# ethan-li-coding/AD-Census

Hardware: NVIDIA H100
Metric: disparity-maps/sec (450x375x64) (higher is better)
Workload: dtype f32

## Files before the change

### adcensus_b200/csrc/adc_common.cuh

```cuda
#pragma once
#include <cuda.h>
#include <cuda_runtime.h>
#include <stdint.h>

#include "img_format.h"

#define ADC_INVALID_F (__int_as_float(0x7f800000))
#define ADC_LARGE_F 99999.0f
#define ADC_CNT 16

struct AdcDims {
    int W, H, D, Dp;
    int dmin, dmax;
    int N;
    long long vol_stride;
};

struct AdcParams {
    AdcDims dm;
    int L1, L2, t1, t2;
    float p1, p2, p1_4, p2_4, p1_10, p2_10;
    int tso;
    int irv_ts; float irv_th;
    float lr_thres;
// ... 34 lines not shown
}
inline void adc_once_done(AdcOnce& o) {
    int dev = 0;
    cudaGetDevice(&dev);
    o.done[dev & 63].store(1, std::memory_order_release);
}

inline int adc_sm_count() {
    int dev = 0, n = 0;
    cudaGetDevice(&dev);
    cudaDeviceGetAttribute(&n, cudaDevAttrMultiProcessorCount, dev);
    return n > 0 ? n : 1;
}

struct alignas(64) AdcArmTmaps { unsigned char map[2][2][128]; };
struct alignas(64) AdcSoTmaps { unsigned char cost[2][2][128]; unsigned char rec[2][128]; int T[2], NS[2]; unsigned smem[2]; };
typedef CUresult (*AdcTmapEncodeFn)(CUtensorMap*, CUtensorMapDataType, cuuint32_t, void*, const cuuint64_t*, const cuuint64_t*,
                                    const cuuint32_t*, const cuuint32_t*, CUtensorMapInterleave, CUtensorMapSwizzle,
                                    CUtensorMapL2promotion, CUtensorMapFloatOOBfill);
AdcTmapEncodeFn adc_tmap_encoder();

struct AdcWave {
    int S;
    uint8_t* bgr;
    unsigned* bgrx;
    uint8_t* gray;
    unsigned long long* census;
    float* volA; float* volB;
    uchar4* arms;
    const AdcArmTmaps* arm_tm;
    unsigned* arm_rec;
    uint16_t* sup_h; uint16_t* sup_v;
    uint8_t* dmap;
    float* disp_l; float* disp_r; float* disp_t;
    uint8_t* label; uint8_t* flag;
    int* pend;
    int* vlist;
    int* counters;
    int* rowcnt;
    unsigned* so_bitrows;
    unsigned* so_rec;
    const AdcSoTmaps* so_tm;
    int* vote_work;
    int2* vote_chg;
    uchar2* vote_alr;
    uchar2* vote_atbT;
    int* vote_pslotT;
    uint16_t* vote_val;
    uint8_t* vote_dirtyb;
    int* vote_state;
    int* vote_off;
    unsigned* vote_hist;
    const float* lut_ad;
    const float* lut_cen;
    const double* ray_sin; const double* ray_cos;
    const short2* ray_off;
};
// ... 42 lines not shown
                        const uint16_t* sup, cudaStream_t st, unsigned long long* launches);
void adc_launch_arm_sum2(const AdcParams& P, const AdcWave& w, const float* src, float* dst, int dir,
                         const uint16_t* sup_mid, cudaStream_t st, unsigned long long* launches);
bool adc_cost_arm_sum_h_available(const AdcParams& P);
bool adc_launch_cost_arm_sum_h(const AdcParams& P, const AdcWave& w, float* dst, float* cost_out, cudaStream_t st,
                               unsigned long long* launches);
size_t adc_arm_rec_bytes(const AdcDims& dm, int L1);
bool adc_arm_tmaps_encode(const AdcParams& P, int S, float* volA, float* volB, AdcArmTmaps* out);
size_t adc_arm_overread_floats(const AdcDims& dm);
void adc_launch_so_bitrows(const AdcParams& P, const AdcWave& w, cudaStream_t st, unsigned long long* launches);
size_t adc_so_rec_bytes(const AdcDims& dm);
size_t adc_so_bitrow_bytes(const AdcDims& dm);
bool adc_so_tmaps_encode(const AdcParams& P, int S, float* volA, float* volB, unsigned* so_rec, AdcSoTmaps* out);
int adc_launch_scanline(const AdcParams& P, const AdcWave& w, const float* src, float* dst, int sx, int sy,
                        cudaStream_t st, unsigned long long* launches);
int adc_launch_wta(const AdcParams& P, const AdcWave& w, const float* vol, cudaStream_t st, unsigned long long* launches);
int adc_launch_scanline_wta(const AdcParams& P, const AdcWave& w, const float* src, float* rec, cudaStream_t st,
                            unsigned long long* launches);
int adc_launch_wta_merge(const AdcParams& P, const AdcWave& w, const float* rec, cudaStream_t st, unsigned long long* launches);
void adc_launch_confidence(const AdcParams& P, const AdcWave& w, const float* vol, float* min_cost, float* peak_ratio,
                           cudaStream_t st, unsigned long long* launches);
void adc_launch_outlier(const AdcParams& P, const AdcWave& w, cudaStream_t st, unsigned long long* launches);
void adc_launch_build_lists(const AdcParams& P, const AdcWave& w, cudaStream_t st, unsigned long long* launches);
void adc_launch_active_lists(const AdcParams& P, const AdcWave& w, cudaStream_t st, unsigned long long* launches);
void adc_launch_voting(const AdcParams& P, const AdcWave& w, cudaStream_t st, unsigned long long* launches);
void adc_launch_interp_list(const AdcParams& P, const AdcWave& w, int k, cudaStream_t st, unsigned long long* launches);
void adc_launch_discontinuity(const AdcParams& P, const AdcWave& w, const float* vol, cudaStream_t st, unsigned long long* launches);
int adc_launch_render(const AdcDims& dm, const float* d_disp, unsigned* d_mm, uint8_t* d_gray, uint8_t* d_jet, float* d_mm_out,
                      cudaStream_t st, unsigned long long* launches);
void adc_launch_cloud(const AdcParams& P, const AdcWave& w1, const float* d_disp, const uint8_t* d_bgr, float* d_cloud,
// ... 4 lines not shown
```

### adcensus_b200/csrc/engine.cu

```cuda
#include <cuda_runtime.h>

#include <float.h>
#include <math.h>
#include <stdarg.h>
#include <stddef.h>
#include <stdio.h>
#include <stdlib.h>
#include <string.h>

#include <algorithm>
#include <string>
#include <vector>

#include "../../include/adcensus_b200.h"
#include "adc_common.cuh"
#include "ca_plan.h"
#include "so_plan.h"

static_assert(sizeof(adc_option) == 60, "adc_option must match the reference's ADCensusOption (60 bytes)");
static_assert(offsetof(adc_option, so_p1) == 32 && offsetof(adc_option, irv_th) == 48 &&
              offsetof(adc_option, do_lr_check) == 56 && offsetof(adc_option, do_discontinuity_adjustment) == 58,
              "adc_option field offsets must match adcensus_types.h:45-75");
static_assert(sizeof(adc_image_desc) == 32 && offsetof(adc_image_desc, reserved) == 4 &&
              offsetof(adc_image_desc, row_pitch) == 8 && offsetof(adc_image_desc, plane_pitch) == 16 &&
// ... 123 lines not shown
    t.pend = c.take<int>((size_t)S * 2 * N);
    t.vlist = c.take<int>((size_t)S * 2 * N);
    t.counters = c.take<int>((size_t)S * ADC_CNT);
    t.vote_alr = c.take<uchar2>((size_t)S * N);
    t.vote_chg = c.take<int2>((size_t)S * N);
    t.vote_atbT = c.take<uchar2>((size_t)S * N);
    t.vote_pslotT = c.take<int>((size_t)S * N);
    t.vote_val = c.take<uint16_t>((size_t)S * N);
    t.vote_dirtyb = c.take<uint8_t>((size_t)S * N);
    t.vote_state = c.take<int>((size_t)S * N);
    t.vote_off = c.take<int>((size_t)S * (N + 1));
    t.rowcnt = c.take<int>((size_t)S * 2 * dm.H);
    t.so_bitrows = c.take<unsigned>((size_t)S * adc_so_bitrow_bytes(dm) / 4);
    t.so_rec = c.take<unsigned>((size_t)S * adc_so_rec_bytes(dm) / 4);
    t.vote_work = c.take<int>((size_t)S * N);
    t.vote_hist = reinterpret_cast<unsigned*>(t.volB);
    if (w) *w = t;
    return c.off;
}

void build_params(adc_engine* e) {
    const adc_option& o = e->opt;
    AdcParams& P = e->P;
    P.dm.W = e->W; P.dm.H = e->H;
    P.dm.dmin = o.min_disparity; P.dm.dmax = o.max_disparity;
    P.dm.D = o.max_disparity - o.min_disparity;
    P.dm.Dp = (P.dm.D + 3) / 4 * 4;
    P.dm.N = e->W * e->H;
    P.dm.vol_stride = (long long)P.dm.N * P.dm.Dp;
    P.L1 = std::min(o.cross_L1, 255);
// ... 209 lines not shown
    }
    if ((rc = launched("aggregation"))) return rc;
    if (ev) CK(cudaEventRecord(ev[2], st));
    if (last_stage <= ADC_STAGE_AGG4) return ADC_OK;

    adc_launch_diffmaps(P, w, st, L);
    adc_launch_so_bitrows(P, w, st, L);
    SoVolumeUse vol_use{};
    for (int i = 0; i < outs.n; i++) vol_use.opt_export |= outs.o[i].stage == ADC_VOL_OPT;
    vol_use.confidence = maps.dst[ADC_MAP_MIN_COST] || maps.dst[ADC_MAP_PEAK_RATIO];
    vol_use.discontinuity = e->opt.do_discontinuity_adjustment != 0;
    vol_use.debug_run = debug_run || last_stage < ADC_STAGE_WTA;
    const int wta_force = (e->cfg.debug_flags & ADC_DBG_UNFUSED_SO_WTA) ? SO_WTA_NEVER
                          : (e->cfg.debug_flags & ADC_DBG_FUSED_SO_WTA) ? SO_WTA_ALWAYS : SO_WTA_AUTO;
    const bool so_wta = so_wta_fused(vol_use, wta_force, P.dm.W, P.dm.H, P.dm.D, P.dm.Dp, P.dm.dmin, P.dm.vol_stride);
    static const int dirs[4][2] = {{1, 0}, {-1, 0}, {0, 1}, {0, -1}};
    for (int ps = 0; ps < 4; ps++) {
        const float* src = (ps % 2 == 0) ? A : B;
        float* dst = (ps % 2 == 0) ? B : A;
        if (ps == 3 && so_wta ? adc_launch_scanline_wta(P, w, src, dst, st, L)
                              : adc_launch_scanline(P, w, src, dst, dirs[ps][0], dirs[ps][1], st, L))
            return fail(ADC_ERR_UNSUPPORTED, "scanline pass not launched (disparity range %d, limit 256)", P.dm.D);
        if (ps % 2 == 0) e->dbg_init = B; else e->dbg_aggr = ps == 3 && so_wta ? nullptr : A;
        if (ps == 3) e->dbg_so_wta = so_wta;
        if (ps == 3) export_vol(ADC_VOL_OPT, A);
        if (stop(ADC_STAGE_SO1 + ps)) return launched("scanline optimisation");
    }
    if ((rc = launched("scanline optimisation"))) return rc;
    if (ev) CK(cudaEventRecord(ev[3], st));

    if (so_wta) adc_launch_wta_merge(P, w, A, st, L);
    else if (adc_launch_wta(P, w, A, st, L)) return fail(ADC_ERR_UNSUPPORTED, "WTA launch failed");
    if (maps.dst[ADC_MAP_WTA_LEFT])
        CK(cudaMemcpyAsync(maps.dst[ADC_MAP_WTA_LEFT], w.disp_l, mapN * sizeof(float), cudaMemcpyDeviceToDevice, st));
    if (maps.dst[ADC_MAP_WTA_RIGHT])
        CK(cudaMemcpyAsync(maps.dst[ADC_MAP_WTA_RIGHT], w.disp_r, mapN * sizeof(float), cudaMemcpyDeviceToDevice, st));
    if (maps.dst[ADC_MAP_MIN_COST] || maps.dst[ADC_MAP_PEAK_RATIO])
        adc_launch_confidence(P, w, A, static_cast<float*>(maps.dst[ADC_MAP_MIN_COST]),
// ... 1331 lines not shown
            case 16:
            case 17: {
                const long long plane = so_wta_plane(P.dm.W, P.dm.H, P.dm.D, P.dm.Dp);
                if (SO_WTA_FIELDS * plane > P.dm.vol_stride)
                    return fail(ADC_ERR_UNSUPPORTED, "adc_profile_kernel: the WTA records do not fit in a pair's volume");
                const double recs = 4.0 * SO_WTA_FIELDS * P.dm.H * (double)so_wta_row_records(P.dm.W, P.dm.D, P.dm.Dp, P.dm.dmin);
                if (kernel_id == 16) {
                    if (adc_launch_scanline_wta(P, w, w.volA, w.volB, ln.st, &e->launches)) return fail(ADC_ERR_UNSUPPORTED, "scanline");
                    bytes = V + 6 * N + recs + 4 * N;
                } else {
                    adc_launch_wta_merge(P, w, w.volB, ln.st, &e->launches);
                    bytes = recs + 4 * N;
                }
                break;
            }
            default: return fail(ADC_ERR_ARG, "adc_profile_kernel: unknown kernel id %d", kernel_id);
        }
    }
    CK(cudaEventRecord(e1, ln.st));
    CK(cudaStreamSynchronize(ln.st));
    float ms = 0;
    CK(cudaEventElapsedTime(&ms, e0, e1));
    *avg_ms = ms / reps;
    if (algorithmic_bytes) *algorithmic_bytes = bytes * e->S;
    return ADC_OK;
}

int adc_debug_run(adc_engine* e, const uint8_t* img_left, const uint8_t* img_right, int32_t last_stage) {
    const char* fn = "adc_debug_run";
    if (!e) return fail(ADC_ERR_ARG, "%s: engine is NULL", fn);
// ... 93 lines not shown
```

### adcensus_b200/csrc/k_scanline.cu

```cuda
#include "adc_common.cuh"
#include "so_plan.h"
#include <cuda.h>
#include <string.h>

template <int K>
struct Piece { static constexpr int G = (K % 4 == 0) ? 4 : ((K % 2 == 0) ? 2 : 1); static constexpr int NP = K / G; };

template <int K>
__device__ __forceinline__ void ld_vec(const float* p, int lane, int Dp, float (&v)[K]) {
    constexpr int G = Piece<K>::G, NP = Piece<K>::NP;
#pragma unroll
    for (int j = 0; j < NP; j++) {
        const int d = lane * K + j * G;
        if (d < Dp) {
            if (G == 4) { const float4 t = *reinterpret_cast<const float4*>(p + d); v[j*G] = t.x; v[j*G+1] = t.y; v[j*G+2] = t.z; v[j*G+3] = t.w; }
            else if (G == 2) { const float2 t = *reinterpret_cast<const float2*>(p + d); v[j*G] = t.x; v[j*G+1] = t.y; }
            else v[j] = p[d];
        } else {
#pragma unroll
            for (int g = 0; g < G; g++) v[j * G + g] = 0.f;
        }
    }
}

// ... 100 lines not shown
}
__device__ __forceinline__ void mbar_wait(unsigned bar, unsigned parity) {
    unsigned ok, spins = 0;
    do {
        asm volatile("{\n\t.reg .pred p;\n\tmbarrier.try_wait.parity.shared::cta.b64 p, [%1], %2;\n\tselp.u32 %0, 1, 0, p;\n\t}"
                     : "=r"(ok) : "r"(bar), "r"(parity) : "memory");
        if (!ok && ++spins > (1u << 24)) __trap();
    } while (!ok);
}
__device__ __forceinline__ void tma_load_4d(unsigned dst, const CUtensorMap* map, int c0, int c1, int c2, int c3, unsigned bar) {
    asm volatile("cp.async.bulk.tensor.4d.shared::cluster.global.tile.mbarrier::complete_tx::bytes [%0], [%1, {%2, %3, %4, %5}], [%6];"
                 ::"r"(dst), "l"(reinterpret_cast<unsigned long long>(map)), "r"(c0), "r"(c1), "r"(c2), "r"(c3), "r"(bar)
                 : "memory");
}

template <int K, int LPS, bool FULL, bool WTA>
__device__ __forceinline__ void so_pass(const CUtensorMap& tm_cost, const CUtensorMap& tm_rec, const AdcParams& P,
                                        float* __restrict__ dst, float* __restrict__ disp_l, int sx, int sy, int T, int NS) {
    constexpr int LPW = 32 / LPS;
    if constexpr (WTA) { sx = 0; sy = -1; }
    extern __shared__ __align__(128) unsigned char so_smem[];
    const AdcDims& dm = P.dm;
    const int lane = threadIdx.x & 31, wid = threadIdx.x >> 5;
    const int sub = lane / LPS, gl = lane % LPS;
    const int line0 = (blockIdx.x * SO_WARPS + wid) * LPW;
    const int line = line0 + sub;
    const int pair = blockIdx.y;
    const int n_lines = sx ? dm.H : dm.W, n_steps = sx ? dm.W : dm.H;
    if (line0 >= n_lines) return;
    const bool live = line < n_lines;
// ... 150 lines not shown
    }
#pragma unroll
    for (int o = LPS / 2; o >= 1; o >>= 1) minL = fminf(minL, __shfl_xor_sync(0xffffffffu, minL, o));
    if constexpr (WTA) {
        wta_left(row, L, minL, 0);
        wta_advance(0);
    }

    for (int step = 1; step < n_steps; step++) {
        float C[K];
        bool a1;
        unsigned bits;
        row = fetch(C, a1, bits);
        pi += pstep;

        const float up = __shfl_up_sync(0xffffffffu, L[K - 1], 1, LPS);
        const float down = __shfl_down_sync(0xffffffffu, L[0], 1, LPS);
        const float left_in = gl == 0 ? ADC_LARGE_F : up;
        const float right_in = gl == LPS - 1 ? ADC_LARGE_F : down;
        const float P1a = a1 ? P.p1 : P.p1_4, P1b = a1 ? P.p1_4 : P.p1_10;
        const float P2a = a1 ? P.p2 : P.p2_4, P2b = a1 ? P.p2_4 : P.p2_10;
        const float m4a = __fadd_rn(minL, P2a), m4b = __fadd_rn(minL, P2b);

        float Ln[K];
        float mn = ADC_LARGE_F;
#pragma unroll
        for (int k = 0; k < K; k++) {
            const bool a2 = (bits >> k) & 1u;
            const float P1 = a2 ? P1a : P1b;
            const float l1 = L[k];
            const float l2 = __fadd_rn(k > 0 ? L[k - 1] : left_in, P1);
            const float l3 = __fadd_rn(k < K - 1 ? L[k + 1] : right_in, P1);
            const float l4 = a2 ? m4a : m4b;
            float v = __fadd_rn(C[k], fminf(fminf(l1, l2), fminf(l3, l4)));
            v = __fmul_rn(v, 0.5f);
            Ln[k] = v;
            if (valid[k]) mn = fminf(mn, v);
        }
        if constexpr (WTA) {
            if constexpr (FULL && K == 8) {
                const int b = (gl >> 2) & 1;
                const float4 lo = make_float4(Ln[0], Ln[1], Ln[2], Ln[3]), hi = make_float4(Ln[4], Ln[5], Ln[6], Ln[7]);
                *reinterpret_cast<float4*>(row + 8 * gl + 4 * b) = b ? hi : lo;
                *reinterpret_cast<float4*>(row + 8 * gl + 4 - 4 * b) = b ? lo : hi;
            } else st_vec<K>(row, gl, Dp, Ln);
        } else if (live) st_vec<K>(O + (size_t)pi * Dp, gl, Dp, Ln);
#pragma unroll
        for (int k = 0; k < K; k++) L[k] = valid[k] ? Ln[k] : ADC_LARGE_F;
#pragma unroll
        for (int o = LPS / 2; o >= 1; o >>= 1) mn = fminf(mn, __shfl_xor_sync(0xffffffffu, mn, o));
        minL = mn;
        if constexpr (WTA) {
            wta_left(row, Ln, mn, step);
// ... 2 lines not shown
    }
}

template <int K, int LPS, bool FULL>
__global__ void __launch_bounds__(SO_WARPS * 32, SO_MIN_CTAS)
k_scanline(const __grid_constant__ CUtensorMap tm_cost, const __grid_constant__ CUtensorMap tm_rec, AdcParams P,
           float* __restrict__ dst, int sx, int sy, int T, int NS) {
    so_pass<K, LPS, FULL, false>(tm_cost, tm_rec, P, dst, nullptr, sx, sy, T, NS);
}

template <int K, int LPS, bool FULL>
__global__ void __launch_bounds__(SO_WARPS * 32, SO_MIN_CTAS)
k_scanline_wta(const __grid_constant__ CUtensorMap tm_cost, const __grid_constant__ CUtensorMap tm_rec, AdcParams P,
               float* __restrict__ rec, float* __restrict__ disp_l, int T, int NS) {
    so_pass<K, LPS, FULL, true>(tm_cost, tm_rec, P, rec, disp_l, 0, -1, T, NS);
}

template <int K, int LPS, bool FULL>
constexpr bool so_wta_built() { return LPS != 32 && !(K == 1 && FULL); }

template <int K, int LPS, bool FULL, bool WTA>
static int launch_scanline_kf(const AdcParams& P, const AdcWave& w, const CUtensorMap& tc, const CUtensorMap& tr,
                              int T, int NS, size_t smem, float* dst, int sx, int sy, cudaStream_t st) {
    if constexpr (WTA && !so_wta_built<K, LPS, FULL>()) {
        return 1;
    } else {
        constexpr int LPW = 32 / LPS;
        const int n_lines = sx ? P.dm.H : P.dm.W;
        const void* fn;
        if constexpr (WTA) fn = (const void*)k_scanline_wta<K, LPS, FULL>;
// ... 45 lines not shown
                    CU_TENSOR_MAP_SWIZZLE_NONE, CU_TENSOR_MAP_L2_PROMOTION_L2_256B, CU_TENSOR_MAP_FLOAT_OOB_FILL_NONE) != CUDA_SUCCESS)
                return false;
            memcpy(out->cost[v][axis], &tm, 128);
        }
        {
            const cuuint64_t gdim[4] = {(cuuint64_t)nrec, (cuuint64_t)dm.W, (cuuint64_t)dm.H, (cuuint64_t)S * 4};
            const cuuint64_t gstr[3] = {(cuuint64_t)nrec * 4, (cuuint64_t)dm.W * nrec * 4, (cuuint64_t)dm.N * nrec * 4};
            const cuuint32_t box[4] = {(cuuint32_t)nrec, bx, by, 1};
            CUtensorMap tm;
            if (enc(&tm, CU_TENSOR_MAP_DATA_TYPE_UINT32, 4, so_rec, gdim, gstr, box, estr, CU_TENSOR_MAP_INTERLEAVE_NONE,
                    CU_TENSOR_MAP_SWIZZLE_NONE, CU_TENSOR_MAP_L2_PROMOTION_L2_256B, CU_TENSOR_MAP_FLOAT_OOB_FILL_NONE) != CUDA_SUCCESS)
                return false;
            memcpy(out->rec[axis], &tm, 128);
        }
    }
    return true;
}

template <bool WTA>
static int launch_scanline(const AdcParams& P, const AdcWave& w, const float* src, float* dst, int sx, int sy,
                           cudaStream_t st, unsigned long long* launches) {
    const int Dp = P.dm.Dp;
    if (Dp > 256 || !w.so_tm || (src != w.volA && src != w.volB)) return 1;
    const int axis = sx ? 0 : 1;
    CUtensorMap tc, tr;
    memcpy(&tc, w.so_tm->cost[src == w.volB ? 1 : 0][axis], 128);
    memcpy(&tr, w.so_tm->rec[axis], 128);
    const int T = w.so_tm->T[axis], NS = w.so_tm->NS[axis];
    const size_t smem = w.so_tm->smem[axis];
    int rc = 1;
#define SO_GO(KK, LL) rc = (P.dm.D == KK * LL ? launch_scanline_kf<KK, LL, true, WTA>(P, w, tc, tr, T, NS, smem, dst, sx, sy, st) \
                                                  : launch_scanline_kf<KK, LL, false, WTA>(P, w, tc, tr, T, NS, smem, dst, sx, sy, st))
    switch (so_lanes_per_line(Dp)) {
        case 8:
            switch ((Dp + 7) / 8) { case 1: SO_GO(1, 8); break; case 2: SO_GO(2, 8); break; case 3: SO_GO(3, 8); break; case 4: SO_GO(4, 8); break;
                                    case 5: SO_GO(5, 8); break; case 6: SO_GO(6, 8); break; case 7: SO_GO(7, 8); break; default: SO_GO(8, 8); }
            break;
        case 16:
            switch ((Dp + 15) / 16) { case 5: SO_GO(5, 16); break; case 6: SO_GO(6, 16); break; case 7: SO_GO(7, 16); break; default: SO_GO(8, 16); }
            break;
        default:
            switch ((Dp + 31) / 32) { case 5: SO_GO(5, 32); break; case 6: SO_GO(6, 32); break; case 7: SO_GO(7, 32); break; default: SO_GO(8, 32); }
    }
#undef SO_GO
    if (rc) return rc;
    ++*launches;
    return 0;
}

int adc_launch_scanline(const AdcParams& P, const AdcWave& w, const float* src, float* dst, int sx, int sy,
                        cudaStream_t st, unsigned long long* launches) {
    return launch_scanline<false>(P, w, src, dst, sx, sy, st, launches);
}

int adc_launch_scanline_wta(const AdcParams& P, const AdcWave& w, const float* src, float* rec, cudaStream_t st,
                            unsigned long long* launches) {
    return launch_scanline<true>(P, w, src, rec, 0, -1, st, launches);
}

size_t adc_so_rec_bytes(const AdcDims& dm) { return (size_t)4 * dm.N * so_rec_words(dm.Dp) * 4; }
size_t adc_so_bitrow_bytes(const AdcDims& dm) { return (size_t)4 * dm.H * so_row_words(dm.W) * 4; }
```

### adcensus_b200/csrc/so_plan.h

```cpp
#pragma once
#include <stddef.h>

#ifdef __CUDACC__
#define SO_HD __host__ __device__
#else
#define SO_HD
#endif

#define SO_WARPS 4
#define SO_MIN_CTAS 8
#define SO_SMEM_MAX (160 * 1024)

SO_HD inline int so_rec_words(int Dp) { return ((1 + (Dp + 31) / 32 + 1) + 3) / 4 * 4; }
SO_HD inline int so_lanes_per_line(int Dp) { return Dp <= 64 ? 8 : (Dp <= 128 ? 16 : 32); }
SO_HD inline unsigned so_region(unsigned bytes) { return (bytes + 127u) / 128u * 128u; }
SO_HD inline unsigned so_cost_region(int Dp, int T) { return so_region((unsigned)(T * (32 / so_lanes_per_line(Dp)) * Dp * 4)); }
SO_HD inline unsigned so_slot_bytes(int Dp, int T) {
    return so_cost_region(Dp, T) + so_region((unsigned)(T * (32 / so_lanes_per_line(Dp)) * so_rec_words(Dp) * 4));
}
inline size_t so_smem_bytes(int Dp, int T, int NS) { return (size_t)SO_WARPS * NS * (so_slot_bytes(Dp, T) + 8); }

struct SoPlan { int T, NS; size_t smem; int ctas, ctas_per_sm, waves; };

inline SoPlan so_plan(int W, int H, int Dp, int S, int axis_y, int sm_count, size_t smem_per_sm, size_t smem_reserved_per_cta) {
// ... 5 lines not shown
        SoPlan p{};
        p.T = c[0]; p.NS = c[1];
        p.smem = so_smem_bytes(Dp, p.T, p.NS);
        if (p.smem > SO_SMEM_MAX) continue;
        p.ctas_per_sm = (int)(smem_per_sm / (p.smem + smem_reserved_per_cta));
        if (p.ctas_per_sm > SO_MIN_CTAS) p.ctas_per_sm = SO_MIN_CTAS;
        if (p.ctas_per_sm < 1) continue;
        p.ctas = (n_lines + lines_per_cta - 1) / lines_per_cta * S;
        const int resident = p.ctas_per_sm * sm_count;
        p.waves = (p.ctas + resident - 1) / resident;
        if (best.T == 0 || p.waves < best.waves) best = p;
    }
    return best;
}

#define SO_WTA_FIELDS 6
SO_HD inline int so_wta_band(int Dp) { return SO_WARPS * (32 / so_lanes_per_line(Dp)); }
SO_HD inline int so_wta_slots(int Dp, int D) { return so_wta_band(Dp) + D - 1; }
inline long long so_wta_plane(int W, int H, int D, int Dp) {
    const int c = so_wta_band(Dp);
    return (long long)H * ((W + c - 1) / c) * so_wta_slots(Dp, D);
}
inline long long so_wta_row_records(int W, int D, int Dp, int dmin) {
    const int c = so_wta_band(Dp);
    long long n = 0;
    for (int x0 = 0; x0 < W; x0 += c) {
        const int lo = x0 - dmin - (D - 1) > 0 ? x0 - dmin - (D - 1) : 0;
        const int xe = x0 + c < W ? x0 + c : W;
        const int hi = xe - 1 - dmin < W - 1 ? xe - 1 - dmin : W - 1;
        if (hi >= lo) n += hi - lo + 1;
// ... 21 lines not shown
```

### adcensus_b200/engine.py

```python
from __future__ import annotations

import ctypes
from pathlib import Path

import numpy as np

Invalid_Float = float("inf")

STAGES = ["COST", "ARMS", "AGG1", "AGG2", "AGG3", "AGG4", "SO1", "SO2", "SO3", "SO4",
          "WTA", "OUTLIER", "VOTE", "INTERP", "DISC", "MEDIAN"]
STAGE = {n: i for i, n in enumerate(STAGES)}
TAPS = ["GRAY_L", "GRAY_R", "CENSUS_L", "CENSUS_R", "VOL_INIT", "VOL_AGGR", "ARMS", "SUPCNT_H",
        "SUPCNT_V", "DISP_L", "DISP_R", "MISMATCHES", "OCCLUSIONS"]
TAP = {n: i for i, n in enumerate(TAPS)}
_TAP_DTYPE = {"GRAY_L": np.uint8, "GRAY_R": np.uint8, "CENSUS_L": np.uint64, "CENSUS_R": np.uint64,
              "VOL_INIT": np.float32, "VOL_AGGR": np.float32, "ARMS": np.uint8, "SUPCNT_H": np.uint16,
              "SUPCNT_V": np.uint16, "DISP_L": np.float32, "DISP_R": np.float32,
              "MISMATCHES": np.int32, "OCCLUSIONS": np.int32}


class ADCensusOption(ctypes.Structure):
    _fields_ = [("min_disparity", ctypes.c_int32), ("max_disparity", ctypes.c_int32),
                ("lambda_ad", ctypes.c_int32), ("lambda_census", ctypes.c_int32),
                ("cross_L1", ctypes.c_int32), ("cross_L2", ctypes.c_int32),
# ... 10 lines not shown
            if k not in dict(self._fields_):
                raise AttributeError(f"ADCensusOption has no field {k!r}")
            setattr(self, k, v)


assert ctypes.sizeof(ADCensusOption) == 60


class _Config(ctypes.Structure):
    _fields_ = [("device", ctypes.c_int32), ("wave_pairs", ctypes.c_int32), ("lanes", ctypes.c_int32),
                ("debug_flags", ctypes.c_int32), ("reserved", ctypes.c_int32 * 12)]


DBG_NO_RAY_TABLE, DBG_VOTE_ENUM, DBG_VOTE_GLOBAL_STATE, DBG_UNFUSED_AGG, DBG_POISON = 1, 2, 4, 8, 16
DBG_UNFUSED_SO_WTA, DBG_FUSED_SO_WTA = 32, 64


def poison_flags(byte: int) -> int:
    return DBG_POISON | ((int(byte) & 0xff) << 8)

COST_HWD, COST_DHW = 0, 1
COST_F32, COST_F16, COST_BF16 = 0, 1, 2
COST_MAX = 65536.0
COST_LAYOUTS = {"hwd": COST_HWD, "dhw": COST_DHW}
COST_DTYPES = {"f32": COST_F32, "f16": COST_F16, "bf16": COST_BF16}

VOL_COST, VOL_AGGR, VOL_OPT = 0, 1, 2
VOL_STAGES = {"cost": VOL_COST, "aggr": VOL_AGGR, "opt": VOL_OPT}
_VOL_NP = {COST_F32: np.float32, COST_F16: np.float16, COST_BF16: np.uint16}

# ... 621 lines not shown
    def synchronize(self):
        _check(self._L.adc_synchronize(self._h))

    @property
    def launch_count(self) -> int:
        return int(self._L.adc_launch_count(self._h))

    def last_stage_ms(self):
        out = (ctypes.c_float * 6)()
        _check(self._L.adc_last_stage_ms(self._h, ctypes.byref(out)))
        return list(out)

    PROFILE_KERNELS = {"cost_volume": 0, "arm_sum_h": 1, "arm_sum_v_div": 2, "scanline_x": 3, "scanline_y": 4, "wta": 5,
                       "arm_sum2_v": 6, "arm_sum2_h": 7, "arm_sum_h_div": 8, "arm_sum_v": 9, "cost_ingest": 10,
                       "cost_export": 11, "confidence": 12, "image_ingest": 13,
                       "rectify": 14, "cost_arm_sum_h": 15, "scanline_y_wta": 16, "wta_merge": 17}

    def profile_kernel(self, name: str, reps: int = 5):
        ms, by = ctypes.c_float(), ctypes.c_double()
        _check(self._L.adc_profile_kernel(self._h, self.PROFILE_KERNELS[name], reps, ctypes.byref(ms), ctypes.byref(by)))
        return ms.value, by.value

    def set_pipelined(self, on: bool = True):
        _check(self._L.adc_set_pipelined(self._h, 1 if on else 0))

    def join(self, stream: int = 0):
        _check(self._L.adc_join(self._h, stream))

    def render_disparity(self, disp: np.ndarray):
        disp = np.ascontiguousarray(disp, np.float32).reshape(self.height, self.width)
        gray = np.empty((self.height, self.width), np.uint8)
# ... 82 lines not shown
```

### include/adcensus_b200.h

```cpp
#ifndef ADCENSUS_B200_H_
#define ADCENSUS_B200_H_

#include <stddef.h>
#include <stdint.h>

#ifdef __cplusplus
extern "C" {
#endif

typedef struct adc_option {
    int32_t min_disparity;
    int32_t max_disparity;
    int32_t lambda_ad;
    int32_t lambda_census;
    int32_t cross_L1;
    int32_t cross_L2;
    int32_t cross_t1;
    int32_t cross_t2;
    float   so_p1;
    float   so_p2;
    int32_t so_tso;
    int32_t irv_ts;
    float   irv_th;
    float   lrcheck_thres;
// ... 16 lines not shown
typedef struct adc_config {
    int32_t device;
    int32_t wave_pairs;
    int32_t lanes;
    int32_t debug_flags;
    int32_t reserved[12];
} adc_config;

enum {
    ADC_DBG_NO_RAY_TABLE = 1,
    ADC_DBG_VOTE_ENUM = 2,
    ADC_DBG_VOTE_GLOBAL_STATE = 4,
    ADC_DBG_UNFUSED_AGG = 8,
    ADC_DBG_UNFUSED_SO_WTA = 32,
    ADC_DBG_FUSED_SO_WTA = 64,
    ADC_DBG_POISON = 16
};
#define ADC_DBG_POISON_BYTE(b) (((b) & 0xff) << 8)

void adc_default_option(adc_option* opt);

#define ADC_MAX_DISPARITY_RANGE 256
#define ADC_MAX_HEIGHT 4096
#define ADC_MAX_WIDTH 10000

int adc_create(int32_t width, int32_t height, const adc_option* opt, const adc_config* cfg, adc_engine** out);

void adc_destroy(adc_engine* e);

int adc_match(adc_engine* e, const uint8_t* img_left, const uint8_t* img_right, float* disp_left);
// ... 200 lines not shown
```

Before: 2033.

## Fuse backward-x and forward-y scanline passes into one wavefront kernel

Adds a k_scanline_xy kernel that runs the second horizontal scanline pass and the first vertical pass together. Each warp takes a column strip and walks it with TMA-fed shared-memory ring buffers. The vertical state for each strip column stays in shared memory, and horizontal carries pass between strips through global memory with acquire/release flags. This removes one full read and write of the cost volume and one kernel launch. In exchange it serialises work across strips through spin-waits and lowers parallelism to strips×pairs warps, and it is used only when 8 lanes per line are chosen and the pipeline runs past SO3.

After: 2084, median of 6. 2.5% higher.

```diff
diff --git a/adcensus_b200/csrc/adc_common.cuh b/adcensus_b200/csrc/adc_common.cuh
--- a/adcensus_b200/csrc/adc_common.cuh
+++ b/adcensus_b200/csrc/adc_common.cuh
@@ -72,7 +72,7 @@
 }
 
 struct alignas(64) AdcArmTmaps { unsigned char map[2][2][128]; };
-struct alignas(64) AdcSoTmaps { unsigned char cost[2][2][128]; unsigned char rec[2][128]; int T[2], NS[2]; unsigned smem[2]; };
+struct alignas(64) AdcSoTmaps { unsigned char cost[2][2][128]; unsigned char rec[2][128]; int T[2], NS[2]; unsigned smem[2]; int xy_NS, xy_Wc; unsigned xy_smem; };
 typedef CUresult (*AdcTmapEncodeFn)(CUtensorMap*, CUtensorMapDataType, cuuint32_t, void*, const cuuint64_t*, const cuuint64_t*,
                                     const cuuint32_t*, const cuuint32_t*, CUtensorMapInterleave, CUtensorMapSwizzle,
                                     CUtensorMapL2promotion, CUtensorMapFloatOOBfill);
@@ -99,6 +99,7 @@
     unsigned* so_bitrows;
     unsigned* so_rec;
     const AdcSoTmaps* so_tm;
+    unsigned* so_xy_ws;
     int* vote_work;
     int2* vote_chg;
     uchar2* vote_alr;
@@ -171,6 +172,7 @@
 bool adc_so_tmaps_encode(const AdcParams& P, int S, float* volA, float* volB, unsigned* so_rec, AdcSoTmaps* out);
 int adc_launch_scanline(const AdcParams& P, const AdcWave& w, const float* src, float* dst, int sx, int sy,
                         cudaStream_t st, unsigned long long* launches);
+int adc_launch_scanline_xy(const AdcParams& P, const AdcWave& w, cudaStream_t st, unsigned long long* launches);
 int adc_launch_wta(const AdcParams& P, const AdcWave& w, const float* vol, cudaStream_t st, unsigned long long* launches);
 int adc_launch_scanline_wta(const AdcParams& P, const AdcWave& w, const float* src, float* rec, cudaStream_t st,
                             unsigned long long* launches);
diff --git a/adcensus_b200/csrc/engine.cu b/adcensus_b200/csrc/engine.cu
--- a/adcensus_b200/csrc/engine.cu
+++ b/adcensus_b200/csrc/engine.cu
@@ -161,6 +161,7 @@
     t.so_bitrows = c.take<unsigned>((size_t)S * adc_so_bitrow_bytes(dm) / 4);
     t.so_rec = c.take<unsigned>((size_t)S * adc_so_rec_bytes(dm) / 4);
     t.vote_work = c.take<int>((size_t)S * N);
+    t.so_xy_ws = c.take<unsigned>((size_t)so_xy_ws_words(dm.W, S));
     t.vote_hist = reinterpret_cast<unsigned*>(t.volB);
     if (w) *w = t;
     return c.off;
@@ -400,14 +401,22 @@
     const int wta_force = (e->cfg.debug_flags & ADC_DBG_UNFUSED_SO_WTA) ? SO_WTA_NEVER
                           : (e->cfg.debug_flags & ADC_DBG_FUSED_SO_WTA) ? SO_WTA_ALWAYS : SO_WTA_AUTO;
     const bool so_wta = so_wta_fused(vol_use, wta_force, P.dm.W, P.dm.H, P.dm.D, P.dm.Dp, P.dm.dmin, P.dm.vol_stride);
+    const int xy_force = (e->cfg.debug_flags & ADC_DBG_UNFUSED_SO_XY) ? SO_XY_NEVER
+                         : (e->cfg.debug_flags & ADC_DBG_FUSED_SO_XY) ? SO_XY_ALWAYS : SO_XY_AUTO;
+    SoXyPlan xy_plan{};
+    if (w.so_tm && w.so_tm->xy_NS) { xy_plan.T = w.so_tm->T[0]; xy_plan.NS = w.so_tm->xy_NS; xy_plan.Wc = w.so_tm->xy_Wc; }
+    const bool so_xy = so_xy_fused(last_stage > ADC_STAGE_SO3, last_stage >= ADC_STAGE_SO3, xy_force, P.dm.Dp, xy_plan);
     static const int dirs[4][2] = {{1, 0}, {-1, 0}, {0, 1}, {0, -1}};
     for (int ps = 0; ps < 4; ps++) {
         const float* src = (ps % 2 == 0) ? A : B;
         float* dst = (ps % 2 == 0) ? B : A;
+        if (so_xy && ps == 1) continue;
         if (ps == 3 && so_wta ? adc_launch_scanline_wta(P, w, src, dst, st, L)
-                              : adc_launch_scanline(P, w, src, dst, dirs[ps][0], dirs[ps][1], st, L))
+            : so_xy && ps == 2 ? adc_launch_scanline_xy(P, w, st, L)
+                               : adc_launch_scanline(P, w, src, dst, dirs[ps][0], dirs[ps][1], st, L))
             return fail(ADC_ERR_UNSUPPORTED, "scanline pass not launched (disparity range %d, limit 256)", P.dm.D);
         if (ps % 2 == 0) e->dbg_init = B; else e->dbg_aggr = ps == 3 && so_wta ? nullptr : A;
+        if (ps == 2 && so_xy) e->dbg_aggr = nullptr;
         if (ps == 3) e->dbg_so_wta = so_wta;
         if (ps == 3) export_vol(ADC_VOL_OPT, A);
         if (stop(ADC_STAGE_SO1 + ps)) return launched("scanline optimisation");
@@ -1769,6 +1778,11 @@
                 }
                 break;
             }
+            case 18:
+                if (adc_launch_scanline_xy(P, w, ln.st, &e->launches)) return fail(ADC_ERR_UNSUPPORTED, "scanline");
+                bytes = 2 * V + 2 * 4.0 * N * so_rec_words(P.dm.Dp) +
+                        2 * 4.0 * so_xy_carry_floats(P.dm.W, P.dm.H, P.dm.Dp, w.so_tm->xy_Wc);
+                break;
             default: return fail(ADC_ERR_ARG, "adc_profile_kernel: unknown kernel id %d", kernel_id);
         }
     }
diff --git a/adcensus_b200/csrc/k_scanline.cu b/adcensus_b200/csrc/k_scanline.cu
--- a/adcensus_b200/csrc/k_scanline.cu
+++ b/adcensus_b200/csrc/k_scanline.cu
@@ -2,6 +2,7 @@
 #include "so_plan.h"
 #include <cuda.h>
 #include <string.h>
+#include <type_traits>
 
 template <int K>
 struct Piece { static constexpr int G = (K % 4 == 0) ? 4 : ((K % 2 == 0) ? 2 : 1); static constexpr int NP = K / G; };
@@ -138,6 +139,33 @@
                  : "memory");
 }
 
+template <int K, int LPS>
+__device__ __forceinline__ float so_step(const AdcParams& P, const float (&L)[K], float minL, const float (&C)[K], bool a1,
+                                         unsigned bits, const bool (&valid)[K], int gl, float (&Ln)[K]) {
+    const float up = __shfl_up_sync(0xffffffffu, L[K - 1], 1, LPS);
+    const float down = __shfl_down_sync(0xffffffffu, L[0], 1, LPS);
+    const float left_in = gl == 0 ? ADC_LARGE_F : up;
+    const float right_in = gl == LPS - 1 ? ADC_LARGE_F : down;
+    const float P1a = a1 ? P.p1 : P.p1_4, P1b = a1 ? P.p1_4 : P.p1_10;
+    const float P2a = a1 ? P.p2 : P.p2_4, P2b = a1 ? P.p2_4 : P.p2_10;
+    const float m4a = __fadd_rn(minL, P2a), m4b = __fadd_rn(minL, P2b);
+    float mn = ADC_LARGE_F;
+#pragma unroll
+    for (int k = 0; k < K; k++) {
+        const bool a2 = (bits >> k) & 1u;
+        const float P1 = a2 ? P1a : P1b;
+        const float l1 = L[k];
+        const float l2 = __fadd_rn(k > 0 ? L[k - 1] : left_in, P1);
+        const float l3 = __fadd_rn(k < K - 1 ? L[k + 1] : right_in, P1);
+        const float l4 = a2 ? m4a : m4b;
+        float v = __fadd_rn(C[k], fminf(fminf(l1, l2), fminf(l3, l4)));
+        v = __fmul_rn(v, 0.5f);
+        Ln[k] = v;
+        if (valid[k]) mn = fminf(mn, v);
+    }
+    return mn;
+}
+
 template <int K, int LPS, bool FULL, bool WTA>
 __device__ __forceinline__ void so_pass(const CUtensorMap& tm_cost, const CUtensorMap& tm_rec, const AdcParams& P,
                                         float* __restrict__ dst, float* __restrict__ disp_l, int sx, int sy, int T, int NS) {
@@ -318,29 +346,8 @@
         row = fetch(C, a1, bits);
         pi += pstep;
 
-        const float up = __shfl_up_sync(0xffffffffu, L[K - 1], 1, LPS);
-        const float down = __shfl_down_sync(0xffffffffu, L[0], 1, LPS);
-        const float left_in = gl == 0 ? ADC_LARGE_F : up;
-        const float right_in = gl == LPS - 1 ? ADC_LARGE_F : down;
-        const float P1a = a1 ? P.p1 : P.p1_4, P1b = a1 ? P.p1_4 : P.p1_10;
-        const float P2a = a1 ? P.p2 : P.p2_4, P2b = a1 ? P.p2_4 : P.p2_10;
-        const float m4a = __fadd_rn(minL, P2a), m4b = __fadd_rn(minL, P2b);
-
         float Ln[K];
-        float mn = ADC_LARGE_F;
-#pragma unroll
-        for (int k = 0; k < K; k++) {
-            const bool a2 = (bits >> k) & 1u;
-            const float P1 = a2 ? P1a : P1b;
-            const float l1 = L[k];
-            const float l2 = __fadd_rn(k > 0 ? L[k - 1] : left_in, P1);
-            const float l3 = __fadd_rn(k < K - 1 ? L[k + 1] : right_in, P1);
-            const float l4 = a2 ? m4a : m4b;
-            float v = __fadd_rn(C[k], fminf(fminf(l1, l2), fminf(l3, l4)));
-            v = __fmul_rn(v, 0.5f);
-            Ln[k] = v;
-            if (valid[k]) mn = fminf(mn, v);
-        }
+        float mn = so_step<K, LPS>(P, L, minL, C, a1, bits, valid, gl, Ln);
         if constexpr (WTA) {
             if constexpr (FULL && K == 8) {
                 const int b = (gl >> 2) & 1;
@@ -373,6 +380,176 @@
 k_scanline_wta(const __grid_constant__ CUtensorMap tm_cost, const __grid_constant__ CUtensorMap tm_rec, AdcParams P,
                float* __restrict__ rec, float* __restrict__ disp_l, int T, int NS) {
     so_pass<K, LPS, FULL, true>(tm_cost, tm_rec, P, rec, disp_l, 0, -1, T, NS);
+}
+
+__device__ __forceinline__ unsigned ld_acquire_gpu(const unsigned* p) {
+    unsigned v;
+    asm volatile("ld.acquire.gpu.global.u32 %0, [%1];" : "=r"(v) : "l"(p) : "memory");
+    return v;
+}
+__device__ __forceinline__ void st_release_gpu(unsigned* p, unsigned v) {
+    asm volatile("st.release.gpu.global.u32 [%0], %1;" ::"l"(p), "r"(v) : "memory");
+}
+
+template <int K, int LPS, bool FULL>
+__global__ void __launch_bounds__(SO_XY_WARPS * 32, 1)
+k_scanline_xy(const __grid_constant__ CUtensorMap tm_cost, const __grid_constant__ CUtensorMap tm_rec, AdcParams P,
+              float* __restrict__ vol, float* __restrict__ carry, unsigned* __restrict__ ws, int S, int T, int NS, int Wc) {
+    constexpr int LPW = 32 / LPS;
+    extern __shared__ __align__(128) unsigned char so_smem[];
+    const AdcDims& dm = P.dm;
+    const int lane = threadIdx.x & 31, wid = threadIdx.x >> 5;
+    const int sub = lane / LPS, gl = lane % LPS;
+    const int W = dm.W, H = dm.H, D = FULL ? K * LPS : dm.D, Dp = FULL ? K * LPS : dm.Dp;
+    const int strips = (W + Wc - 1) / Wc;
+    unsigned item = 0;
+    if (lane == 0) item = atomicAdd(ws, 1u);
+    item = __shfl_sync(0xffffffffu, item, 0);
+    if (item >= (unsigned)(strips * S)) return;
+    const int j = (int)item / S, pair = (int)item - j * S;
+    const int xe = W - j * Wc;
+    const int ncols = min(Wc, xe);
+    const int nb = (H + LPW - 1) / LPW, cpb = Wc / T, nq = nb * cpb;
+    const int nrec = so_rec_words(Dp);
+    const unsigned cost_region = so_cost_region(Dp, T), rec_region = so_xy_rec_region(Dp, T);
+    const unsigned slot_bytes = so_xy_slot_bytes(Dp, T);
+    unsigned char* wring = so_smem + (size_t)wid * NS * slot_bytes;
+    float* colL = reinterpret_cast<float*>(so_smem + (size_t)SO_XY_WARPS * NS * slot_bytes + (size_t)wid * so_xy_col_bytes(Dp, Wc));
+    float* colM = colL + (size_t)Wc * Dp;
+    const unsigned bar0 = so_smem_u32(so_smem + (size_t)SO_XY_WARPS * (NS * slot_bytes + so_xy_col_bytes(Dp, Wc))) + (unsigned)(wid * NS) * 8u;
+    const unsigned tx = (unsigned)(T * LPW * (Dp + 2 * nrec) * 4);
+
+    auto issue = [&](int q) {
+        const int s = q % NS;
+        const unsigned bar = bar0 + 8u * (unsigned)s, d0 = so_smem_u32(wring + (size_t)s * slot_bytes);
+        const int x0 = xe - (q % cpb + 1) * T, y0 = q / cpb * LPW;
+        mbar_expect_tx(bar, tx);
+        tma_load_4d(d0, &tm_cost, 0, x0, y0, pair, bar);
+        tma_load_4d(d0 + cost_region, &tm_rec, 0, x0, y0, pair * 4 + 1, bar);
+        tma_load_4d(d0 + cost_region + rec_region, &tm_rec, 0, x0, y0, pair * 4 + 2, bar);
+    };
+    if (lane == 0) {
+        for (int s = 0; s < NS; s++) mbar_init(bar0 + 8u * s, 1);
+        asm volatile("fence.mbarrier_init.release.cluster;" ::: "memory");
+        for (int q = 0; q < NS && q < nq; q++) issue(q);
+    }
+    __syncwarp();
+
+    bool valid[K];
+#pragma unroll
+    for (int k = 0; k < K; k++) valid[k] = FULL || (gl * K + k) < D;
+    auto group_min = [&](float m) {
+#pragma unroll
+        for (int o = LPS / 2; o >= 1; o >>= 1) m = fminf(m, __shfl_xor_sync(0xffffffffu, m, o));
+        return m;
+    };
+
+    float* cbase = carry + (size_t)pair * dm.vol_stride;
+    const unsigned* done_prev = ws + 1 + (size_t)(j > 0 ? j - 1 : 0) * S + pair;
+    unsigned* done_mine = ws + 1 + (size_t)j * S + pair;
+    unsigned seen = 0;
+    float cy[K], cymin = ADC_LARGE_F;
+    auto load_carry = [&](int b) {
+        unsigned spins = 0, ns = 32;
+        while (seen < (unsigned)(b + 1)) {
+            seen = ld_acquire_gpu(done_prev);
+            if (seen >= (unsigned)(b + 1)) break;
+            __nanosleep(ns);
+            if (ns < 1024) ns *= 2;
+            if (++spins > (1u << 22)) __trap();
+        }
+        const int y = b * LPW + sub;
+        if (y < H) ld_vec<K>(cbase + ((size_t)(j - 1) * H + y) * Dp, gl, Dp, cy);
+        float m = ADC_LARGE_F;
+#pragma unroll
+        for (int k = 0; k < K; k++) {
+            if (!valid[k] || y >= H) cy[k] = ADC_LARGE_F;
+            m = fminf(m, cy[k]);
+        }
+        cymin = group_min(m);
+    };
+    if (j > 0) load_carry(0);
+
+    const int bit0 = gl * K;
+    const int nsteps = nq * T + LPW - 1;
+    const int cpf = min(4, Wc - LPW);
+    float Lx[K], mx = ADC_LARGE_F;
+#pragma unroll
+    for (int k = 0; k < K; k++) Lx[k] = ADC_LARGE_F;
+    float* V = vol + (size_t)pair * dm.vol_stride;
+    for (int s = 0; s < nsteps; s++) {
+        if (s % T == 0 && s < nq * T) mbar_wait(bar0 + 8u * (unsigned)((s / T) % NS), (unsigned)((s / T / NS) & 1));
+        const int g = s - sub;
+        const bool act = g >= 0 && g < nq * T;
+        const int gg = act ? g : 0;
+        const int q = gg / T, pos = gg - q * T, b = gg / Wc, col = gg - b * Wc;
+        const int y = b * LPW + sub, x = xe - 1 - col;
+        const bool live = act && y < H && col < ncols;
+        const unsigned char* sl = wring + (size_t)(q % NS) * slot_bytes;
+        const int row = sub * T + (T - 1 - pos);
+        float C[K];
+        ld_vec<K>(reinterpret_cast<const float*>(sl) + row * Dp, gl, Dp, C);
+        const unsigned* rx = reinterpret_cast<const unsigned*>(sl + cost_region) + row * nrec;
+        const unsigned* ry = reinterpret_cast<const unsigned*>(sl + cost_region + rec_region) + row * nrec;
+        const bool a1x = rx[0] != 0u, a1y = ry[0] != 0u;
+        const unsigned bitsx = __funnelshift_r(rx[1 + (bit0 >> 5)], rx[2 + (bit0 >> 5)], bit0 & 31);
+        const unsigned bitsy = __funnelshift_r(ry[1 + (bit0 >> 5)], ry[2 + (bit0 >> 5)], bit0 & 31);
+
+        const bool head = col == 0;
+        float Lp[K], X[K];
+#pragma unroll
+        for (int k = 0; k < K; k++) Lp[k] = head ? cy[k] : Lx[k];
+        float m = so_step<K, LPS>(P, Lp, head ? cymin : mx, C, a1x, bitsx, valid, gl, X);
+        if (j == 0 && head) {
+            m = ADC_LARGE_F;
+#pragma unroll
+            for (int k = 0; k < K; k++) {
+                X[k] = C[k];
+                if (valid[k]) m = fminf(m, C[k]);
+            }
+        }
+        mx = group_min(m);
+#pragma unroll
+        for (int k = 0; k < K; k++) Lx[k] = valid[k] ? X[k] : ADC_LARGE_F;
+
+        float* cl = colL + (size_t)col * Dp;
+        float Yp[K], Y[K];
+        ld_vec<K>(cl, gl, Dp, Yp);
+#pragma unroll
+        for (int k = 0; k < K; k++) Yp[k] = valid[k] ? Yp[k] : ADC_LARGE_F;
+        m = so_step<K, LPS>(P, Yp, colM[col], X, a1y, bitsy, valid, gl, Y);
+        if (y == 0) {
+            m = ADC_LARGE_F;
+#pragma unroll
+            for (int k = 0; k < K; k++) {
+                Y[k] = X[k];
+                if (valid[k]) m = fminf(m, X[k]);
+            }
+        }
+        m = group_min(m);
+        if (live) st_vec<K>(V + ((size_t)y * W + x) * Dp, gl, Dp, Y);
+        if (act) {
+#pragma unroll
+            for (int k = 0; k < K; k++) Yp[k] = valid[k] ? Y[k] : ADC_LARGE_F;
+            st_vec<K>(cl, gl, Dp, Yp);
+            if (gl == 0) colM[col] = m;
+        }
+        if (live && col == Wc - 1 && j + 1 < strips) st_vec<K>(cbase + ((size_t)j * H + y) * Dp, gl, Dp, Lx);
+        __syncwarp();
+
+        const int gd = s - (LPW - 1);
+        if (gd >= 0 && (gd + 1) % T == 0) {
+            asm volatile("fence.proxy.async.shared::cta;" ::: "memory");
+            __syncwarp();
+            if (lane == 0 && gd / T + NS < nq) issue(gd / T + NS);
+        }
+        if (j + 1 < strips && gd >= 0 && (gd + 1) % Wc == 0) {
+            __threadfence();
+            __syncwarp();
+            if (lane == 0) st_release_gpu(done_mine, (unsigned)(gd / Wc + 1));
+        }
+        if (j > 0 && s % Wc == Wc - 1 - cpf && s / Wc + 1 < nb) load_carry(s / Wc + 1);
+    }
 }
 
 template <int K, int LPS, bool FULL>
@@ -448,7 +625,26 @@
             memcpy(out->rec[axis], &tm, 128);
         }
     }
+    const SoXyPlan xp = so_xy_plan(dm.W, dm.H, Dp, S, adc_sm_count(), (size_t)smem_sm, (size_t)smem_res);
+    if (xp.T == out->T[0]) { out->xy_NS = xp.NS; out->xy_Wc = xp.Wc; out->xy_smem = (unsigned)xp.smem; }
     return true;
+}
+
+template <typename F>
+static int so_dispatch(int D, int Dp, F&& go) {
+    using std::integral_constant;
+#define SO_GO(KK, LL) return D == KK * LL ? go(integral_constant<int, KK>(), integral_constant<int, LL>(), std::true_type()) \
+                                          : go(integral_constant<int, KK>(), integral_constant<int, LL>(), std::false_type())
+    switch (so_lanes_per_line(Dp)) {
+        case 8:
+            switch ((Dp + 7) / 8) { case 1: SO_GO(1, 8); case 2: SO_GO(2, 8); case 3: SO_GO(3, 8); case 4: SO_GO(4, 8);
+                                    case 5: SO_GO(5, 8); case 6: SO_GO(6, 8); case 7: SO_GO(7, 8); default: SO_GO(8, 8); }
+        case 16:
+            switch ((Dp + 15) / 16) { case 5: SO_GO(5, 16); case 6: SO_GO(6, 16); case 7: SO_GO(7, 16); default: SO_GO(8, 16); }
+        default:
+            switch ((Dp + 31) / 32) { case 5: SO_GO(5, 32); case 6: SO_GO(6, 32); case 7: SO_GO(7, 32); default: SO_GO(8, 32); }
+    }
+#undef SO_GO
 }
 
 template <bool WTA>
@@ -462,26 +658,39 @@
     memcpy(&tr, w.so_tm->rec[axis], 128);
     const int T = w.so_tm->T[axis], NS = w.so_tm->NS[axis];
     const size_t smem = w.so_tm->smem[axis];
-    int rc = 1;
-#define SO_GO(KK, LL) rc = (P.dm.D == KK * LL ? launch_scanline_kf<KK, LL, true, WTA>(P, w, tc, tr, T, NS, smem, dst, sx, sy, st) \
-                                                  : launch_scanline_kf<KK, LL, false, WTA>(P, w, tc, tr, T, NS, smem, dst, sx, sy, st))
-    switch (so_lanes_per_line(Dp)) {
-        case 8:
-            switch ((Dp + 7) / 8) { case 1: SO_GO(1, 8); break; case 2: SO_GO(2, 8); break; case 3: SO_GO(3, 8); break; case 4: SO_GO(4, 8); break;
-                                    case 5: SO_GO(5, 8); break; case 6: SO_GO(6, 8); break; case 7: SO_GO(7, 8); break; default: SO_GO(8, 8); }
-            break;
-        case 16:
-            switch ((Dp + 15) / 16) { case 5: SO_GO(5, 16); break; case 6: SO_GO(6, 16); break; case 7: SO_GO(7, 16); break; default: SO_GO(8, 16); }
-            break;
-        default:
-            switch ((Dp + 31) / 32) { case 5: SO_GO(5, 32); break; case 6: SO_GO(6, 32); break; case 7: SO_GO(7, 32); break; default: SO_GO(8, 32); }
-    }
-#undef SO_GO
+    const int rc = so_dispatch(P.dm.D, Dp, [&](auto Kc, auto LPSc, auto FULLc) {
+        return launch_scanline_kf<decltype(Kc)::value, decltype(LPSc)::value, decltype(FULLc)::value, WTA>(
+            P, w, tc, tr, T, NS, smem, dst, sx, sy, st);
+    });
     if (rc) return rc;
     ++*launches;
     return 0;
 }
 
+int adc_launch_scanline_xy(const AdcParams& P, const AdcWave& w, cudaStream_t st, unsigned long long* launches) {
+    const AdcSoTmaps* tm = w.so_tm;
+    if (P.dm.Dp > 256 || !tm || tm->xy_NS == 0) return 1;
+    const int strips = (P.dm.W + tm->xy_Wc - 1) / tm->xy_Wc, items = strips * w.S;
+    if (cudaMemsetAsync(w.so_xy_ws, 0, (size_t)(1 + items) * sizeof(unsigned), st) != cudaSuccess) return 1;
+    CUtensorMap tc, tr;
+    memcpy(&tc, tm->cost[1][0], 128);
+    memcpy(&tr, tm->rec[0], 128);
+    so_dispatch(P.dm.D, P.dm.Dp, [&](auto Kc, auto LPSc, auto FULLc) {
+        const auto fn = k_scanline_xy<decltype(Kc)::value, decltype(LPSc)::value, decltype(FULLc)::value>;
+        static AdcOnce attr_once;
+        if (adc_once_needed(attr_once)) {
+            cudaFuncSetAttribute((const void*)fn, cudaFuncAttributeMaxDynamicSharedMemorySize, SO_SMEM_MAX);
+            cudaFuncSetAttribute((const void*)fn, cudaFuncAttributePreferredSharedMemoryCarveout, cudaSharedmemCarveoutMaxShared);
+            adc_once_done(attr_once);
+        }
+        fn<<<(items + SO_XY_WARPS - 1) / SO_XY_WARPS, SO_XY_WARPS * 32, tm->xy_smem, st>>>(
+            tc, tr, P, w.volB, w.volA, w.so_xy_ws, w.S, tm->T[0], tm->xy_NS, tm->xy_Wc);
+        return 0;
+    });
+    ++*launches;
+    return 0;
+}
+
 int adc_launch_scanline(const AdcParams& P, const AdcWave& w, const float* src, float* dst, int sx, int sy,
                         cudaStream_t st, unsigned long long* launches) {
     return launch_scanline<false>(P, w, src, dst, sx, sy, st, launches);
diff --git a/adcensus_b200/csrc/so_plan.h b/adcensus_b200/csrc/so_plan.h
--- a/adcensus_b200/csrc/so_plan.h
+++ b/adcensus_b200/csrc/so_plan.h
@@ -43,6 +43,46 @@
     return best;
 }
 
+#define SO_XY_WARPS 4
+#define SO_XY_NS_MAX 8
+SO_HD inline int so_xy_lpw(int Dp) { return 32 / so_lanes_per_line(Dp); }
+SO_HD inline unsigned so_xy_rec_region(int Dp, int T) { return so_region((unsigned)(T * so_xy_lpw(Dp) * so_rec_words(Dp) * 4)); }
+SO_HD inline unsigned so_xy_slot_bytes(int Dp, int T) { return so_cost_region(Dp, T) + 2u * so_xy_rec_region(Dp, T); }
+SO_HD inline unsigned so_xy_col_bytes(int Dp, int Wc) { return so_region((unsigned)(Wc * (Dp + 1) * 4)); }
+SO_HD inline unsigned so_xy_warp_bytes(int Dp, int T, int NS, int Wc) {
+    return (unsigned)NS * so_xy_slot_bytes(Dp, T) + so_xy_col_bytes(Dp, Wc) + 8u * (unsigned)NS;
+}
+inline long long so_xy_ws_words(int W, int S) { return 1 + (long long)S * ((W + 15) / 16); }
+inline long long so_xy_carry_floats(int W, int H, int Dp, int Wc) { return (long long)((W + Wc - 1) / Wc - 1) * H * Dp; }
+
+struct SoXyPlan { int T, NS, Wc, strips, items, ctas; size_t smem; };
+
+inline SoXyPlan so_xy_plan(int W, int H, int Dp, int S, int sm_count, size_t smem_per_sm, size_t smem_reserved_per_cta) {
+    SoXyPlan p{};
+    const SoPlan xp = so_plan(W, H, Dp, S, 0, sm_count, smem_per_sm, smem_reserved_per_cta);
+    if (xp.T == 0) return p;
+    const int T = xp.T, LPW = so_xy_lpw(Dp);
+    const int Wc = (32 + T - 1) / T * T;
+    const int ns_min = (T + LPW - 1 + T - 1) / T;
+    for (int NS = SO_XY_NS_MAX; NS >= ns_min; NS--) {
+        const size_t smem = (size_t)SO_XY_WARPS * so_xy_warp_bytes(Dp, T, NS, Wc);
+        if (smem > SO_SMEM_MAX || smem + smem_reserved_per_cta > smem_per_sm) continue;
+        p.T = T; p.NS = NS; p.Wc = Wc; p.smem = smem;
+        p.strips = (W + Wc - 1) / Wc;
+        p.items = p.strips * S;
+        p.ctas = (p.items + SO_XY_WARPS - 1) / SO_XY_WARPS;
+        return p;
+    }
+    return p;
+}
+
+enum SoXyForce { SO_XY_AUTO = 0, SO_XY_NEVER = 1, SO_XY_ALWAYS = 2 };
+
+inline bool so_xy_fused(bool past_so3, bool reaches_so3, int force, int Dp, const SoXyPlan& plan) {
+    if (force == SO_XY_NEVER || plan.T == 0 || !reaches_so3) return false;
+    return force == SO_XY_ALWAYS || (past_so3 && so_lanes_per_line(Dp) == 8);
+}
+
 #define SO_WTA_FIELDS 6
 SO_HD inline int so_wta_band(int Dp) { return SO_WARPS * (32 / so_lanes_per_line(Dp)); }
 SO_HD inline int so_wta_slots(int Dp, int D) { return so_wta_band(Dp) + D - 1; }
diff --git a/adcensus_b200/engine.py b/adcensus_b200/engine.py
--- a/adcensus_b200/engine.py
+++ b/adcensus_b200/engine.py
@@ -48,6 +48,7 @@
 
 DBG_NO_RAY_TABLE, DBG_VOTE_ENUM, DBG_VOTE_GLOBAL_STATE, DBG_UNFUSED_AGG, DBG_POISON = 1, 2, 4, 8, 16
 DBG_UNFUSED_SO_WTA, DBG_FUSED_SO_WTA = 32, 64
+DBG_UNFUSED_SO_XY, DBG_FUSED_SO_XY = 128, 65536
 
 
 def poison_flags(byte: int) -> int:
@@ -699,7 +700,8 @@
     PROFILE_KERNELS = {"cost_volume": 0, "arm_sum_h": 1, "arm_sum_v_div": 2, "scanline_x": 3, "scanline_y": 4, "wta": 5,
                        "arm_sum2_v": 6, "arm_sum2_h": 7, "arm_sum_h_div": 8, "arm_sum_v": 9, "cost_ingest": 10,
                        "cost_export": 11, "confidence": 12, "image_ingest": 13,
-                       "rectify": 14, "cost_arm_sum_h": 15, "scanline_y_wta": 16, "wta_merge": 17}
+                       "rectify": 14, "cost_arm_sum_h": 15, "scanline_y_wta": 16, "wta_merge": 17,
+                       "scanline_xy": 18}
 
     def profile_kernel(self, name: str, reps: int = 5):
         ms, by = ctypes.c_float(), ctypes.c_double()
diff --git a/include/adcensus_b200.h b/include/adcensus_b200.h
--- a/include/adcensus_b200.h
+++ b/include/adcensus_b200.h
@@ -54,6 +54,8 @@
     ADC_DBG_UNFUSED_AGG = 8,
     ADC_DBG_UNFUSED_SO_WTA = 32,
     ADC_DBG_FUSED_SO_WTA = 64,
+    ADC_DBG_UNFUSED_SO_XY = 128,
+    ADC_DBG_FUSED_SO_XY = 65536,
     ADC_DBG_POISON = 16
 };
 #define ADC_DBG_POISON_BYTE(b) (((b) & 0xff) << 8)
```
